# ivanalberico/End-To-End-Self-Supervised-SLAM

Measured on AMD Instinct MI355X. Metric: online refinement steps/sec @640x480, seq_len=60, higher is better.
Workload: dtype f32

## Files before the change

### end-to-end-self-supervised-slam_amd/csrc/conv.hip

```cpp
#include <cassert>
#include <type_traits>

#include "e2e_common.h"

typedef float f4v __attribute__((ext_vector_type(4)));
typedef float f16v __attribute__((ext_vector_type(16)));

#define CBK 16

enum { ACT_NONE = 0, ACT_RELU = 1, ACT_ELU = 2, ACT_DISP = 3 };

struct ConvArgs {
    const float* src0;
    const float* src1;
    const float* w;
    const float* scale;
    const float* shift;
    const float* res;
    float* out;
    int B, Hs, Ws;
    int Cin, C1, up;
    int Hd, Wd;
    int Ncols, ldw;
    int KH, KW, stride, pad, pad_mode;
// ... 1655 lines not shown
#pragma unroll
            for (int mt = 0; mt < MT; ++mt) av[mt] = ap[ks * 4 * CO + mt * 16];
#pragma unroll
            for (int t = 0; t < 9; ++t) {
                const float bv = bp[((t / 3) * PW + (t % 3)) * 16 + ks * 64];
#pragma unroll
                for (int mt = 0; mt < MT; ++mt) acc[mt * 10 + t] = __builtin_amdgcn_mfma_f32_16x16x4f32(av[mt], bv, acc[mt * 10 + t], 0, 0, 0);
            }
#pragma unroll
            for (int mt = 0; mt < MT; ++mt) acc[mt * 10 + 9] = __builtin_amdgcn_mfma_f32_16x16x4f32(av[mt], one, acc[mt * 10 + 9], 0, 0, 0);
        }
    }
    float* red = smem;
    static_assert(2 * NA * 4 * 64 <= PH * PW * 16 + TH * TW * CO, "reduction scratch");
    __syncthreads();
    if (wave >= 2) {
#pragma unroll
        for (int t = 0; t < NA; ++t)
#pragma unroll
            for (int i = 0; i < 4; ++i) red[((wave - 2) * NA * 4 + t * 4 + i) * 64 + lane] = acc[t][i];
    }
    __syncthreads();
    if (wave < 2) {
#pragma unroll
        for (int t = 0; t < NA; ++t)
#pragma unroll
            for (int i = 0; i < 4; ++i) acc[t][i] += red[(wave * NA * 4 + t * 4 + i) * 64 + lane];
    }
    __syncthreads();
    if (wave == 1) {
#pragma unroll
        for (int t = 0; t < NA; ++t)
#pragma unroll
            for (int i = 0; i < 4; ++i) red[(t * 4 + i) * 64 + lane] = acc[t][i];
    }
    __syncthreads();
    if (wave != 0) return;
    const int64_t sid = ((int64_t)b * gridDim.y + blockIdx.y) * a.nxg + blockIdx.x;
    float* slab = a.slabs + sid * CO * a.npad;
    const int kconv = 9 * a.Cin, cg0 = hf * 16;
#pragma unroll
    for (int mt = 0; mt < MT; ++mt)
#pragma unroll
        for (int t = 0; t < 10; ++t)
#pragma unroll
            for (int i = 0; i < 4; ++i) {
                const float v = acc[mt * 10 + t][i] + red[((mt * 10 + t) * 4 + i) * 64 + lane];
                const int co = mt * 16 + 4 * kq + i;
                if (t < 9) slab[co * a.npad + t * a.Cin + cg0 + l16] = v;
                else if (a.has_bias && hf == 0 && l16 == 0) slab[co * a.npad + kconv] = v;
            }
}

struct StemWgradArgs {
    const float* dz;
    const float* src;
    float* slabs;
    int B, Hs, Ws, Hd, Wd, tiles_x, nxg;
    float in_sub, in_mul;
};

__global__ __launch_bounds__(256) void k_wgrad7x7_stem(StemWgradArgs a) {
    constexpr int TH = 4, TW = 32, PH = 2 * TH + 6, PW = 2 * TW + 5, ROW = 208, NPAD = 148;
    __shared__ float patch[PH * ROW];
    __shared__ float dzs[TH * TW * 64];
    const int tid = threadIdx.x, lane = tid & 63, wave = tid >> 6, l16 = lane & 15, kq = lane >> 4;
    const int y0 = blockIdx.y * TH, b = blockIdx.z;
    int offn[10];
#pragma unroll
    for (int nt = 0; nt < 10; ++nt) {
        const int k = 16 * nt + l16;
        offn[nt] = k + (k / 21) * (ROW - 21) + 48 * kq;
    }
    f4v acc[10];
#pragma unroll
    for (int nt = 0; nt < 10; ++nt) acc[nt] = (f4v){0.f, 0.f, 0.f, 0.f};
    const float* sb = a.src + (int64_t)b * a.Hs * a.Ws * 3;
    const float* zb = a.dz + (int64_t)b * a.Hd * a.Wd * 64;
    for (int tx = 0; tx < a.tiles_x; ++tx) {
        const int x0 = (blockIdx.x * a.tiles_x + tx) * TW;
        if (x0 >= a.Wd) break;
        __syncthreads();
        for (int idx = tid; idx < PH * ROW; idx += 256) {
            const int py = idx / ROW, e = idx - py * ROW;
            const int Y = 2 * y0 - 3 + py, X = 2 * x0 - 3 + e / 3;
            const bool ok = e < 3 * PW && Y >= 0 && Y < a.Hs && X >= 0 && X < a.Ws;
            patch[idx] = ok ? (sb[((int64_t)Y * a.Ws + X) * 3 + (e - (e / 3) * 3)] - a.in_sub) * a.in_mul : 0.f;
        }
        for (int idx = tid; idx < TH * TW * 16; idx += 256) {
            const int q = idx & 15, pix = idx >> 4;
            const int r = pix / TW, x = pix - r * TW;
            const bool ok = y0 + r < a.Hd && x0 + x < a.Wd;
            *(f4v*)&dzs[pix * 64 + q * 4] = ok ? *(const f4v*)(zb + ((int64_t)(y0 + r) * a.Wd + x0 + x) * 64 + q * 4) : (f4v){0.f, 0.f, 0.f, 0.f};
        }
        __syncthreads();
#pragma unroll 1
        for (int r = 0; r < TH; ++r) {
            const float* ap = dzs + (r * TW + 8 * kq) * 64 + 16 * wave + l16;
            const float* bp = patch + 2 * r * ROW;
#pragma unroll 2
            for (int ks = 0; ks < TW / 4; ++ks) {
                const float av = ap[ks * 64];
#pragma unroll
                for (int nt = 0; nt < 10; ++nt) acc[nt] = __builtin_amdgcn_mfma_f32_16x16x4f32(av, bp[offn[nt] + ks * 6], acc[nt], 0, 0, 0);
            }
        }
// ... 632 lines not shown
#pragma unroll
            for (int kw = 0; kw < 3; ++kw) {
                const float* wt = &sw[(kh * 3 + kw) * HC + cq * 4];
                const float gg = head_dz_gather(gz, h, ww, kh, kw, H, W, rya, ryb, rxa, rxb);
#pragma unroll
                for (int c = 0; c < 4; ++c) da[c] = fmaf(gg, wt[c], da[c]);
            }
        if (dact) {
#pragma unroll
            for (int e = 0; e < 4; ++e) da[e] *= act_deriv(xv[e], dact);
        }
        *(f4v*)(dx + n * HC + cq * 4) = da;
    }
#pragma unroll
    for (int k = 0; k < 36; ++k) {
        float v = acc[k];
#pragma unroll
        for (int o = 4; o < 64; o <<= 1) v += __shfl_xor(v, o, 64);
        acc[k] = v;
    }
#pragma unroll
    for (int o = 4; o < 64; o <<= 1) sb += __shfl_xor(sb, o, 64);
    if (lane < 4) {
#pragma unroll
        for (int t = 0; t < 9; ++t)
#pragma unroll
            for (int c = 0; c < 4; ++c) red[wave][t * HC + lane * 4 + c] = acc[t * 4 + c];
        if (lane == 0) red[wave][9 * HC] = sb;
    }
    __syncthreads();
    if (threadIdx.x < 9 * HC + 1)
        partials[(int64_t)blockIdx.x * (9 * HC + 1) + threadIdx.x] = ((red[0][threadIdx.x] + red[1][threadIdx.x]) + red[2][threadIdx.x]) + red[3][threadIdx.x];
}

__global__ __launch_bounds__(256) void k_head_wreduce(const float* __restrict__ partials, int nparts, float* __restrict__ dw, float* __restrict__ dbias) {
    __shared__ float red[4];
    const int col = blockIdx.x;
    float s = 0.f;
    for (int i = threadIdx.x; i < nparts; i += 256) s += partials[(int64_t)i * (9 * HC + 1) + col];
    const float t = block_sum(s, red);
    if (threadIdx.x == 0) {
        if (col == 9 * HC) { if (dbias) dbias[0] = t; }
        else { const int tap = col / HC, ci = col - tap * HC; dw[ci * 9 + tap] = t; }
    }
}

static inline int egrid(int64_t n) { int64_t g = (n + 255) / 256; return (int)(g < 1 ? 1 : (g > 4096 ? 4096 : g)); }

struct GemmCfg { int bm, bn, S; };
#define WGRAD_TARGET 1024

#define CONV_TILE_SHAPES(X)                                                                                      \
    X(64, 64, 2, 2, 1, 1, 32) X(128, 64, 2, 2, 2, 1, 32) X(128, 128, 2, 2, 2, 2, 16) X(128, 32, 4, 1, 1, 1, 32) \
    X(32, 128, 1, 4, 1, 1, 32) X(32, 64, 1, 2, 1, 1, 32) X(64, 32, 2, 1, 1, 1, 32) X(32, 32, 1, 1, 1, 1, 32)
static int tile_max_cb(int bm, int bn) {
#define X(BM, BN, WM, WN, TM, TN, MAXCB) if (bm == BM && bn == BN) return MAXCB;
    CONV_TILE_SHAPES(X)
#undef X
    return 0;
}
static void demote_cb16_only(GemmCfg& c) { if (tile_max_cb(c.bm, c.bn) == 16) c.bn = 64; }

static GemmCfg choose_cfg(int64_t rows, int cols, int K, int cb, bool allow_split, GemmCfg force = GemmCfg{0, 0, 0}) {
    if (force.bm) { GemmCfg f = force; if (!allow_split && f.S > 1) f.S = 1; if (cb != 16) demote_cb16_only(f); return f; }
    GemmCfg c = {64, 64, 1};
    if (cols >= 128) { c.bm = 32; c.bn = 128; }
    if (cols <= 32) {
        c.bm = 128; c.bn = 32;
        if (((rows + 127) / 128) * ((cols + 31) / 32) < 600) c.bm = 64;
    }
    if (allow_split && cols > 32) {
        const int64_t tiles = ((rows + c.bm - 1) / c.bm) * ((cols + c.bn - 1) / c.bn);
        const int nchunks = (K + cb - 1) / cb;
        const int depth = nchunks * cb / 32;
        int S = tiles >= 500 ? 1 : depth < 30 ? 1 : depth < 60 ? 3 : depth < 120 ? 4 : 6;
        while (S < 12 && tiles * S < 200 && (nchunks / (S + 1)) * cb >= 288) ++S;
        while (S > 1 && tiles * S > 1300) --S;
        while (S > 1 && (nchunks / S) * cb < 288) --S;
        if (S < 1) S = 1;
        auto model = [&](int s) {
            const double wgs = (double)tiles * s, per_cu = wgs <= 256 ? 1 : wgs <= 512 ? 2 : wgs <= 768 ? 3 : 0;
            const double f = per_cu == 1 ? 1.0 : per_cu == 2 ? 1.76 : per_cu == 3 ? 2.41 : 2.41 * wgs / 768.0;
            return f * ((double)nchunks / s + 6.0) + (s > 1 ? 4.0 : 0.0);
        };
        if (tiles < 500 && S > 1) {
            int best = S;
            for (int s = S - 2; s <= S + 2; ++s) {
                if (s < 2 || s > 12 || s == S || (nchunks / s) * cb < 288 || tiles * s > 1300) continue;
                if (model(s) < 0.93 * model(best)) best = s;
            }
            S = best;
        }
        c.S = S;
    }
    return c;
}

template <bool TR>
static void launch_tile(ConvArgs& a, int cb, GemmCfg c, dim3 g, hipStream_t st) {
#define X(BM, BN, WM, WN, TM, TN, MAXCB)                                                                                                 \
    if (c.bm == BM && c.bn == BN) {                                                                                                      \
        if constexpr (MAXCB == 32)                                                                                                       \
            if (cb == 32) { hipLaunchKernelGGL((k_conv_gemm<WM, WN, TM, TN, 4, TR, 32>), g, dim3(64 * WM * WN), 0, st, a); return; }     \
        hipLaunchKernelGGL((k_conv_gemm<WM, WN, TM, TN, 4, TR, 16>), g, dim3(64 * WM * WN), 0, st, a);                                   \
        return;                                                                                                                          \
    }
    CONV_TILE_SHAPES(X)
#undef X
    assert(!"launch_tile: shape not in CONV_TILE_SHAPES");
}

template <bool TR>
static void launch_streamk(ConvArgs& a, int cb, int G, float* workspace, hipStream_t st) {
    const int64_t Ntot = (int64_t)a.B * a.Hd * a.Wd;
    SkArgs s;
    s.flags = (unsigned*)workspace;
    s.slabs = workspace + SK_FLAG_FLOATS;
    s.tiles_n = (a.Ncols + 63) / 64;
    s.C = a.KH * a.KW * a.Cin / cb;
    s.I = ((Ntot + 63) / 64) * s.tiles_n * (long long)s.C;
    if (G > SK_MAX_G) G = SK_MAX_G;
    if ((long long)G > s.I) G = (int)s.I;
    s.G = G;
    if (cb == 32) hipLaunchKernelGGL((k_conv_gemm_sk<TR, 32>), dim3(G), dim3(256), 0, st, a, s);
    else hipLaunchKernelGGL((k_conv_gemm_sk<TR, 16>), dim3(G), dim3(256), 0, st, a, s);
}

enum GemmKind { GK_SCALAR, GK_STREAMK, GK_TILE };
enum GemmTail { GT_NONE, GT_SPLITK4, GT_SPLITK, GT_CLS };
struct GemmLaunch { GemmKind kind; GemmTail tail; GemmCfg c; int cb; dim3 g; int G; };

#define CLS_TAP_SLICES 4
static int64_t cls_rows(int B, int Hd, int Wd) { return (int64_t)B * ((Hd + 1) / 2) * ((Wd + 1) / 2); }
static int64_t cls_slab_floats(int B, int Hd, int Wd, int cols) { return CLS_TAP_SLICES * 4 * cls_rows(B, Hd, Wd) * cols; }

template <bool TR>
static GemmLaunch plan_gemm(ConvArgs& a, int vec, float* workspace_all, GemmCfg force) {
    GemmLaunch p{GK_TILE, GT_NONE, GemmCfg{0, 0, 0}, 16, dim3(1), 0};
    const int64_t Ntot = (int64_t)a.B * a.Hd * a.Wd;
    const int K = a.KH * a.KW * a.Cin;
    const int cb = (vec == 4 && a.Cin % 32 == 0 && (a.C1 == a.Cin || a.C1 % 32 == 0)) ? 32 : 16;
    float* workspace = workspace_all ? workspace_all + SK_FLAG_FLOATS : nullptr;
    a.ksplit = 1; a.cps = 0; a.slab = workspace;
    a.bytes0 = (int64_t)a.B * (a.Hs / a.up) * (a.Ws / a.up) * a.C1 * 4;
    a.bytes1 = (int64_t)a.B * a.Hs * a.Ws * (a.Cin - a.C1) * 4;
    a.bytesw = (int64_t)K * a.ldw * 4;
// ... 509 lines not shown
        return p;
    if (vec == 4 && stride == 1 && pad == 1 && Ho == Hs && Wo == Ws && (up == 1 || up == 2) && Hs % up == 0 && Ws % up == 0 && (C1 == Cin || (has_src1 && C1 % 32 == 0)) &&
        getenv("E2E_WGRAD_TAPS") != nullptr && getenv("E2E_WGRAD_TAPS")[0] == '1' && (p = plan(WP_TAPS)).open)
        return p;
    return lean && (p = plan(WP_GEMM16)).open ? p : plan(lean ? WP_GEMM_LEAN : WP_GEMM);
}

int64_t e2e_conv2d_wgrad_workspace_floats(int B, int Ho, int Wo, int Cin, int Cout, int KH, int KW, int has_bias) {
    GEOM_WGRAD_QUERY(g);
    return wgrad_workspace_floats(g, has_bias, false, WGRAD_TARGET);
}

struct WgradOut { float* dw; float* dbias; const float* out_scale; int accumulate; e2e_wgrad_reduce_desc* defer; };

static void wgrad_reduce(const WgradArgs& a, const WgradOut& o, int S, int Mpad, int Npad, int zl, hipStream_t st) {
    if (o.defer) {
        *o.defer = e2e_wgrad_reduce_desc{a.slabs, o.dw, o.dbias, o.out_scale, S, Mpad, Npad, a.Cout, a.Cin, a.KH, a.KW, a.has_bias, o.accumulate, zl, 0};
        return;
    }
    const int64_t tq = (int64_t)a.Cout * ((a.Ngemm + 3) / 4);
    if (zl == 8)
        hipLaunchKernelGGL((k_wgrad_reduce<8>), dim3(egrid(tq * 4)), dim3(512), 0, st, a.slabs, S, Mpad, Npad, a.Cout, a.Cin, a.KH, a.KW, a.has_bias, o.dw,
                           o.dbias, o.accumulate, o.out_scale);
    else
        hipLaunchKernelGGL((k_wgrad_reduce<2>), dim3(egrid(tq * 4)), dim3(128), 0, st, a.slabs, S, Mpad, Npad, a.Cout, a.Cin, a.KH, a.KW, a.has_bias, o.dw,
                           o.dbias, o.accumulate, o.out_scale);
}

enum WgradKernel { WK_DONE, WK_GEMM16, WK_GEMM4_32, WK_GEMM4_64, WK_GEMM_32, WK_GEMM_64 };
struct WgradLaunch { WgradKernel k; dim3 g; int Sz; };

static int wgrad_setup(const WgradIn& in, const ConvGeom& g, int wg_target, const WgradOut& o, hipStream_t st, WgradArgs& a, WgradLaunch& L, bool dry = false) {
    const int B = g.B, Cin = g.Cin, Cout = g.Cout, Ho = g.Ho, Wo = g.Wo;
    const bool tuned = wg_target != 0;
    if (!tuned) wg_target = WGRAD_TARGET;
    L = WgradLaunch{WK_DONE, dim3(1), 0};
    E2E_REQUIRE(in.dz && in.src0 && o.dw && in.workspace && B > 0 && Cin > 0 && Cout > 0, E2E_ERR_ARG, "e2e_conv2d_bwd_weight: bad argument");
    const int vec = (Cin % 4 == 0 && g.C1 % 4 == 0) ? 4 : 1;
    E2E_REQUIRE(vec == 4 || (g.C1 == Cin && g.up == 1 && g.pad_mode == 0), E2E_ERR_ARG, "e2e_conv2d_bwd_weight: scalar path takes one full-resolution zero-padded source");
    a = WgradArgs{};
    a.dz = in.dz; a.src0 = in.src0; a.src1 = in.src1; a.slabs = in.workspace;
    a.B = B; a.Hs = g.Hs; a.Ws = g.Ws; a.Cin = Cin; a.C1 = g.C1; a.up = g.up; a.Ho = Ho; a.Wo = Wo; a.Cout = Cout;
    a.KH = g.KH; a.KW = g.KW; a.stride = g.stride; a.pad = g.pad; a.pad_mode = g.pad_mode; a.has_bias = o.dbias ? 1 : 0;
    a.Ngemm = g.KH * g.KW * Cin + a.has_bias;
    const WgradPlan p = wgrad_choose(g, a.has_bias, in.src1 != nullptr, tuned, wg_target);
    const int S = (int)p.S;
    if (dry && (p.path == WP_STEM || p.path == WP_THIN || p.path == WP_TAPS)) return E2E_OK;
    if (p.path == WP_STEM) {
        StemWgradArgs ta{in.dz, in.src0, in.workspace, B, g.Hs, g.Ws, Ho, Wo, 2, p.nxg, g.in_sub, g.in_mul};
        hipLaunchKernelGGL(k_wgrad7x7_stem, dim3(p.nxg, p.ny, B), dim3(256), 0, st, ta);
    } else if (p.path == WP_THIN) {
        ThinWgradArgs ta{in.dz, in.src0, in.src1, in.workspace, B, Ho, Wo, Cin, g.C1, g.up, p.Npad, a.has_bias, p.tiles_x, p.nxg};
        const dim3 tg((unsigned)p.nxg, (unsigned)p.ny, (unsigned)(B * (Cin / 16)));
        if (Cout == 32) hipLaunchKernelGGL((k_wgrad3x3_thin<2>), tg, dim3(256), 0, st, ta);
        else hipLaunchKernelGGL((k_wgrad3x3_thin<1>), tg, dim3(256), 0, st, ta);
    } else if (p.path == WP_TAPS) {
        TapWgradArgs ta{in.dz, in.src0, in.src1, in.workspace, B, Ho, Wo, Cin, g.C1, g.up, Cout, g.pad_mode == 1 ? 1 : 0, a.has_bias,
                        p.Mpad, p.Npad, p.ptx, p.pty, p.nchunks, p.cps};
        const dim3 tg((unsigned)(Cin / 32), (unsigned)(Cout / 32), (unsigned)S);
        if (a.has_bias) hipLaunchKernelGGL(k_wgrad3x3_taps<true>, tg, dim3(TAP_NT), 0, st, ta);
        else hipLaunchKernelGGL(k_wgrad3x3_taps<false>, tg, dim3(TAP_NT), 0, st, ta);
    }
    if (p.path == WP_STEM || p.path == WP_THIN || p.path == WP_TAPS) {
        wgrad_reduce(a, o, S, p.Mpad, p.Npad, (p.path == WP_TAPS && S < 8) ? 2 : 8, st);
        return E2E_OK;
    }
    const bool use16 = p.path == WP_GEMM16, lean = p.path != WP_GEMM;
    a.Mpad = p.Mpad; a.Npad = p.Npad;
    a.in_sub = g.in_sub; a.in_mul = g.in_mul; a.vec = vec;
    const int64_t P = (int64_t)B * Ho * Wo;
    const int cbp = lean ? 32 : CBK;
    a.pix_per_slice = ((P + p.S - 1) / p.S + cbp - 1) / cbp * cbp;
    L.Sz = (int)((P + a.pix_per_slice - 1) / a.pix_per_slice);
    L.g = dim3((unsigned)(a.Npad / p.tn), (unsigned)(a.Mpad / p.tm), (unsigned)L.Sz);
    L.k = use16 ? WK_GEMM16 : lean ? (p.tm == 32 ? WK_GEMM4_32 : WK_GEMM4_64) : (p.tm == 32 ? WK_GEMM_32 : WK_GEMM_64);
    return E2E_OK;
}

static void wgrad_launch_gemm(const WgradArgs& a, const WgradLaunch& L, hipStream_t st) {
    const dim3 g = L.g;
    const bool two = a.src1 != nullptr;
    if (L.k == WK_GEMM16) hipLaunchKernelGGL((k_wgrad_gemm16<10, 32>), g, dim3(256), 0, st, a);
    else if (L.k == WK_GEMM4_32 && two) hipLaunchKernelGGL((k_wgrad_gemm4<1, 4, 32, true>), g, dim3(256), 0, st, a);
    else if (L.k == WK_GEMM4_32) hipLaunchKernelGGL((k_wgrad_gemm4<1, 4, 32, false>), g, dim3(256), 0, st, a);
    else if (L.k == WK_GEMM4_64 && two) hipLaunchKernelGGL((k_wgrad_gemm4<2, 2, 32, true>), g, dim3(256), 0, st, a);
    else if (L.k == WK_GEMM4_64) hipLaunchKernelGGL((k_wgrad_gemm4<2, 2, 32, false>), g, dim3(256), 0, st, a);
    else if (L.k == WK_GEMM_32 && a.vec == 4) hipLaunchKernelGGL((k_wgrad_gemm<1, 4, 4>), g, dim3(256), 0, st, a);
    else if (L.k == WK_GEMM_32) hipLaunchKernelGGL((k_wgrad_gemm<1, 4, 1>), g, dim3(256), 0, st, a);
    else if (L.k == WK_GEMM_64 && a.vec == 4) hipLaunchKernelGGL((k_wgrad_gemm<2, 2, 4>), g, dim3(256), 0, st, a);
    else if (L.k == WK_GEMM_64) hipLaunchKernelGGL((k_wgrad_gemm<2, 2, 1>), g, dim3(256), 0, st, a);
}

static int bwd_weight_impl(const WgradIn& in, const ConvGeom& g, const WgradOut& o, void* stream, int wg_target = 0) {
    const hipStream_t st = (hipStream_t)stream;
    WgradArgs a;
    WgradLaunch L;
    const int rc = wgrad_setup(in, g, wg_target, o, st, a, L);
    if (rc != E2E_OK) return rc;
    if (L.k != WK_DONE) {
        wgrad_launch_gemm(a, L, st);
        wgrad_reduce(a, o, L.Sz, a.Mpad, a.Npad, L.Sz >= 8 ? 8 : 2, st);
    }
    E2E_LAUNCH_CHECK("e2e_conv2d_bwd_weight");
    return E2E_OK;
}

int e2e_conv2d_bwd_weight(const float* dz, const float* src0, const float* src1, int C1, int up, float* dw, float* dbias,
// ... 175 lines not shown
```

### end-to-end-self-supervised-slam_amd/csrc/depth_ops.hip

```cpp
#include "e2e_common.h"

#define DT 256

__device__ __forceinline__ unsigned int f2key(float f) {
    const unsigned int b = __float_as_uint(f);
    return (b & 0x80000000u) ? ~b : (b | 0x80000000u);
}
__device__ __forceinline__ float key2f(unsigned int k) {
    return __uint_as_float((k & 0x80000000u) ? (k & 0x7FFFFFFFu) : ~k);
}

#define MED_BINS 2048
struct MedState {
    unsigned int prefix, rank, key, index, count;
};

__device__ unsigned int select_bin(const unsigned int* __restrict__ hist, int nb, unsigned int r, unsigned int* r_in, unsigned int* sh) {
    unsigned int c[8], s = 0;
#pragma unroll
    for (int j = 0; j < 8; ++j) {
        const int i = threadIdx.x * 8 + j;
        c[j] = (i < nb) ? hist[i] : 0u;
        s += c[j];
    }
    unsigned int x = s;
#pragma unroll
    for (int o = 1; o < 64; o <<= 1) {
        const unsigned int y = __shfl_up(x, o, 64);
        if ((threadIdx.x & 63) >= o) x += y;
    }
    __syncthreads();
    if ((threadIdx.x & 63) == 63) sh[2 + (threadIdx.x >> 6)] = x;
    __syncthreads();
    unsigned int woff = 0;
    for (int w = 0; w < (int)(threadIdx.x >> 6); ++w) woff += sh[2 + w];
    const unsigned int excl = woff + x - s;
    if (r >= excl && r < excl + s) {
        unsigned int acc = excl;
#pragma unroll
        for (int j = 0; j < 8; ++j) {
            if (r < acc + c[j]) { sh[0] = threadIdx.x * 8 + j; sh[1] = r - acc; break; }
            acc += c[j];
        }
    }
    __syncthreads();
    *r_in = sh[1];
    return sh[0];
}

template <int PASS, bool RECIP = false>
__global__ __launch_bounds__(DT) void k_median_hist(const float* __restrict__ x, int64_t n, unsigned int rank0,
                                                    unsigned int* __restrict__ hist , MedState* __restrict__ st,
                                                    float* __restrict__ recip_out = nullptr) {
    __shared__ unsigned int lh[MED_BINS];
    __shared__ unsigned int sh[8];
// ... 26 lines not shown
    for (int i = threadIdx.x; i < MED_BINS; i += DT)
        if (lh[i]) atomicAdd(&gh[i], lh[i]);
}

__global__ __launch_bounds__(DT) void k_median_final(const float* __restrict__ x, int64_t n, const unsigned int* __restrict__ hist,
                                                     MedState* __restrict__ st, float* __restrict__ value_out) {
    __shared__ unsigned int sh[8];
    unsigned int rin;
    const unsigned int b2 = select_bin(hist + 2 * MED_BINS, 1024, st->rank, &rin, sh);
    const unsigned int key = st->prefix | b2;
    if (blockIdx.x == 0 && threadIdx.x == 0) { st->key = key; *value_out = key2f(key); }
    for (int64_t i = (int64_t)blockIdx.x * DT + threadIdx.x; i < n; i += (int64_t)gridDim.x * DT)
        if (f2key(x[i]) == key) { atomicMin(&st->index, (unsigned int)i); atomicAdd(&st->count, 1u); }
}

__global__ __launch_bounds__(DT) void k_median_final_scale(const float* __restrict__ delta, int64_t n, const unsigned int* __restrict__ hist,
                                                           MedState* __restrict__ st, const float* __restrict__ m_gt, float* __restrict__ median_out,
                                                           float* __restrict__ depth, float* __restrict__ ratio_out) {
    __shared__ unsigned int sh[8];
    unsigned int rin;
    const unsigned int b2 = select_bin(hist + 2 * MED_BINS, 1024, st->rank, &rin, sh);
    const unsigned int key = st->prefix | b2;
    const float med = key2f(key);
    const float rho = m_gt[0] / med;
    if (blockIdx.x == 0 && threadIdx.x == 0) {
        st->key = key;
        *median_out = med;
        if (ratio_out) ratio_out[0] = rho;
    }
    for (int64_t i = (int64_t)blockIdx.x * DT + threadIdx.x; i < n; i += (int64_t)gridDim.x * DT) {
        const float d = delta[i];
        depth[i] = d * rho;
        if (f2key(d) == key) { atomicMin(&st->index, (unsigned int)i); atomicAdd(&st->count, 1u); }
    }
}

__global__ void k_median_init(unsigned int* hist, MedState* st) {
    for (int i = threadIdx.x; i < 3 * MED_BINS; i += blockDim.x) hist[i] = 0;
    if (threadIdx.x == 0) { st->prefix = 0; st->rank = 0; st->key = 0; st->index = 0xFFFFFFFFu; st->count = 0; }
}

__global__ __launch_bounds__(DT) void k_dot_partials(const float* __restrict__ a, const float* __restrict__ b, int64_t n,
                                                     float* __restrict__ partials) {
    __shared__ float red[DT / 64];
    float acc = 0.f;
    for (int64_t i = (int64_t)blockIdx.x * DT + threadIdx.x; i < n; i += (int64_t)gridDim.x * DT) acc = fmaf(a[i], b[i], acc);
    const float s = block_sum(acc, red);
    if (threadIdx.x == 0) partials[blockIdx.x] = s;
}

__global__ __launch_bounds__(DT) void k_scale_chain_bwd(const float* __restrict__ g, const float* __restrict__ delta,
                                                        const float* __restrict__ m_gt, const float* __restrict__ m_delta,
                                                        const MedState* __restrict__ st, const float* __restrict__ partials,
                                                        int nparts, float* __restrict__ g_disp, int64_t n, const int* __restrict__ elems, int n_elems) {
    __shared__ float sS;
    if (threadIdx.x == 0) {
        double acc = 0.0;
        for (int i = 0; i < nparts; ++i) acc += (double)partials[i];
        sS = (float)acc;
    }
    __syncthreads();
    const float md = m_delta[0], rho = m_gt[0] / md;
    const float corr = -(rho / md) * sS;
    const float share = corr / (float)(n_elems > 0 ? (unsigned int)n_elems : st->count);
    for (int64_t i = (int64_t)blockIdx.x * DT + threadIdx.x; i < n; i += (int64_t)gridDim.x * DT) {
        const float d = delta[i];
        float gd = rho * g[i];
        if (n_elems > 0) {
            for (int e = 0; e < n_elems; ++e) if ((int)i == elems[e]) gd += share;
        } else if (d == md) gd += share;
        g_disp[i] = -(d * d) * gd;
    }
}

__global__ __launch_bounds__(DT) void k_diff_partials(const float* __restrict__ a, const float* __restrict__ b, int64_t n, int kind,
                                                      float* __restrict__ partials) {
    __shared__ float red[DT / 64];
    float acc = 0.f;
    for (int64_t i = (int64_t)blockIdx.x * DT + threadIdx.x; i < n; i += (int64_t)gridDim.x * DT) {
        const float e = a[i] - b[i];
        acc += (kind == 2) ? e * e : fabsf(e);
    }
    const float s = block_sum(acc, red);
    if (threadIdx.x == 0) partials[blockIdx.x] = s;
}

__global__ void k_sum_partials(const float* __restrict__ partials, int nparts, double scale, float* __restrict__ out) {
    __shared__ double sh[4];
    double acc = 0.0;
    for (int i = threadIdx.x; i < nparts; i += blockDim.x) acc += (double)partials[i];
    acc = wave_sum_d(acc);
    if ((threadIdx.x & 63) == 0) sh[threadIdx.x >> 6] = acc;
    __syncthreads();
    if (threadIdx.x == 0) out[0] = (float)((((sh[0] + sh[1]) + sh[2]) + sh[3]) * scale);
}

__global__ __launch_bounds__(DT) void k_diff_bwd(const float* __restrict__ a, const float* __restrict__ b, const float* __restrict__ g,
                                                 int64_t n, int kind, float* __restrict__ gb) {
    const float s = g[0] / (float)n;
    for (int64_t i = (int64_t)blockIdx.x * DT + threadIdx.x; i < n; i += (int64_t)gridDim.x * DT) {
        const float e = a[i] - b[i];
        gb[i] = (kind == 2) ? s * (-2.f * e) : s * ((e > 0.f) ? -1.f : ((e < 0.f) ? 1.f : 0.f));
    }
}

#define NMET 8
__global__ __launch_bounds__(DT) void k_metrics_partials(const float* __restrict__ gt, const float* __restrict__ pred, int64_t n,
                                                         int mask_zero_gt, float* __restrict__ partials) {
    __shared__ float red[DT / 64];
    float acc[NMET] = {0.f, 0.f, 0.f, 0.f, 0.f, 0.f, 0.f, 0.f};
    for (int64_t i = (int64_t)blockIdx.x * DT + threadIdx.x; i < n; i += (int64_t)gridDim.x * DT) {
// ... 24 lines not shown
        for (int i = 0; i < nparts; ++i) acc += (double)partials[threadIdx.x * nparts + i];
        tot[threadIdx.x] = acc;
    }
    __syncthreads();
    if (threadIdx.x < 7) {
        double v = tot[threadIdx.x] / tot[7];
        if (threadIdx.x == 2 || threadIdx.x == 3) v = sqrt(v);
        out[threadIdx.x] = (float)v;
    }
}

__global__ __launch_bounds__(DT) void k_adam(float* __restrict__ p, const float* __restrict__ g, float* __restrict__ m, float* __restrict__ v,
                                             int64_t n, float one_minus_b1, float b2, float one_minus_b2, float step_size,
                                             float bc2_sqrt, float eps, const float* __restrict__ participants,
                                             const float2* __restrict__ schedule, const int* __restrict__ step_counter, int schedule_len) {
    const int64_t n4 = n >> 2;
    const float cnt = participants ? fmaxf(participants[0], 1.f) : 1.f;
    if (schedule) {
        int t = step_counter[0];
        t = t < 1 ? 1 : (t > schedule_len ? schedule_len : t);
        const float2 sc = schedule[t - 1];
        step_size = sc.x;
        bc2_sqrt = sc.y;
    }
    float4* p4 = (float4*)p; const float4* g4 = (const float4*)g; float4* m4 = (float4*)m; float4* v4 = (float4*)v;
    for (int64_t i = (int64_t)blockIdx.x * DT + threadIdx.x; i < n4; i += (int64_t)gridDim.x * DT) {
        float4 pp = p4[i], gg = g4[i], mm = m4[i], vv = v4[i];
        float* pa = (float*)&pp; float* ga = (float*)&gg; float* ma = (float*)&mm; float* va = (float*)&vv;
#pragma unroll
        for (int k = 0; k < 4; ++k) {
            ga[k] = ga[k] / cnt;
            ma[k] = ma[k] + one_minus_b1 * (ga[k] - ma[k]);
            va[k] = va[k] * b2 + one_minus_b2 * (ga[k] * ga[k]);
            const float den = sqrtf(va[k]) / bc2_sqrt + eps;
            pa[k] = pa[k] - step_size * (ma[k] / den);
        }
        p4[i] = pp; m4[i] = mm; v4[i] = vv;
    }
    for (int64_t i = (n4 << 2) + (int64_t)blockIdx.x * DT + threadIdx.x; i < n; i += (int64_t)gridDim.x * DT) {
        const float gi = g[i] / cnt;
        const float mi = m[i] + one_minus_b1 * (gi - m[i]);
        const float vi = v[i] * b2 + one_minus_b2 * (gi * gi);
        m[i] = mi; v[i] = vi;
        p[i] = p[i] - step_size * (mi / (sqrtf(vi) / bc2_sqrt + eps));
    }
}

__global__ void k_adam_advance(int* __restrict__ step_counter) { step_counter[0] += 1; }

static inline int sgrid(int64_t n, int cap = 1024) {
    int64_t g = (n + DT - 1) / DT;
    return (int)(g < 1 ? 1 : (g > cap ? cap : g));
}
#define RED_PARTS 512

extern "C" {

int64_t e2e_median_workspace_bytes(void) { return (3 * MED_BINS + 8) * 4; }

int e2e_median_lower(const float* x, int64_t n, float* value_out, void* workspace, void* stream) {
    E2E_REQUIRE(n > 0 && n < 0xFFFFFFFFll && x && value_out && workspace, E2E_ERR_ARG, "e2e_median_lower: bad argument");
    hipStream_t st = (hipStream_t)stream;
    unsigned int* hist = (unsigned int*)workspace;
    MedState* ms = (MedState*)(hist + 3 * MED_BINS);
    const unsigned int rank = (unsigned int)((n - 1) / 2);
    const int g = sgrid(n, 96);
    hipLaunchKernelGGL(k_median_init, dim3(1), dim3(256), 0, st, hist, ms);
    hipLaunchKernelGGL(k_median_hist<0>, dim3(g), dim3(DT), 0, st, x, n, rank, hist, ms, (float*)nullptr);
    hipLaunchKernelGGL(k_median_hist<1>, dim3(g), dim3(DT), 0, st, x, n, rank, hist, ms, (float*)nullptr);
    hipLaunchKernelGGL(k_median_hist<2>, dim3(g), dim3(DT), 0, st, x, n, rank, hist, ms, (float*)nullptr);
    hipLaunchKernelGGL(k_median_final, dim3(g), dim3(DT), 0, st, x, n, hist, ms, value_out);
    E2E_LAUNCH_CHECK("e2e_median_lower");
    return E2E_OK;
}

int64_t e2e_depth_scale_workspace_bytes(void) { return e2e_median_workspace_bytes() + RED_PARTS * 4 + 64; }

int e2e_depth_scale_fwd(const float* disp, const float* median_gt, float* delta, float* depth, float* median_delta,
                        float* ratio_out, void* workspace, int64_t n, void* stream) {
    E2E_REQUIRE(n > 0 && disp && median_gt && delta && depth && median_delta && workspace, E2E_ERR_ARG, "e2e_depth_scale_fwd: bad argument");
    hipStream_t st = (hipStream_t)stream;
    E2E_REQUIRE(n < 0xFFFFFFFFll, E2E_ERR_ARG, "e2e_depth_scale_fwd: too many elements");
    unsigned int* hist = (unsigned int*)workspace;
    MedState* ms = (MedState*)(hist + 3 * MED_BINS);
    const unsigned int rank = (unsigned int)((n - 1) / 2);
    const int g = sgrid(n, 96);
    hipLaunchKernelGGL(k_median_init, dim3(1), dim3(256), 0, st, hist, ms);
    hipLaunchKernelGGL((k_median_hist<0, true>), dim3(g), dim3(DT), 0, st, disp, n, rank, hist, ms, delta);
    hipLaunchKernelGGL(k_median_hist<1>, dim3(g), dim3(DT), 0, st, (const float*)delta, n, rank, hist, ms, (float*)nullptr);
    hipLaunchKernelGGL(k_median_hist<2>, dim3(g), dim3(DT), 0, st, (const float*)delta, n, rank, hist, ms, (float*)nullptr);
    hipLaunchKernelGGL(k_median_final_scale, dim3(sgrid(n)), dim3(DT), 0, st, (const float*)delta, n, (const unsigned int*)hist, ms, median_gt, median_delta, depth, ratio_out);
    E2E_LAUNCH_CHECK("e2e_depth_scale_fwd");
    return E2E_OK;
}

__global__ __launch_bounds__(DT) void k_fixed_scale_fwd(const float* __restrict__ disp, float scale, float* __restrict__ delta, float* __restrict__ depth,
                                                        int64_t n) {
    for (int64_t i = (int64_t)blockIdx.x * DT + threadIdx.x; i < n; i += (int64_t)gridDim.x * DT) {
        const float d = 1.f / disp[i];
        if (delta) delta[i] = d;
        depth[i] = d * scale;
    }
}
__global__ __launch_bounds__(DT) void k_fixed_scale_bwd(const float* __restrict__ g_depth, const float* __restrict__ disp, float scale,
                                                        float* __restrict__ g_disp, int64_t n) {
    for (int64_t i = (int64_t)blockIdx.x * DT + threadIdx.x; i < n; i += (int64_t)gridDim.x * DT) {
        const float d = 1.f / disp[i];
        g_disp[i] = -(g_depth[i] * scale) * d * d;
    }
}

int e2e_depth_fixed_scale_fwd(const float* disp, float scale, float* delta, float* depth, int64_t n, void* stream) {
    E2E_REQUIRE(n > 0 && disp && depth, E2E_ERR_ARG, "e2e_depth_fixed_scale_fwd: bad argument");
    hipLaunchKernelGGL(k_fixed_scale_fwd, dim3(sgrid(n)), dim3(DT), 0, (hipStream_t)stream, disp, scale, delta, depth, n);
    E2E_LAUNCH_CHECK("e2e_depth_fixed_scale_fwd");
    return E2E_OK;
}

int e2e_depth_fixed_scale_bwd(const float* g_depth, const float* disp, float scale, float* g_disp, int64_t n, void* stream) {
    E2E_REQUIRE(n > 0 && g_depth && disp && g_disp, E2E_ERR_ARG, "e2e_depth_fixed_scale_bwd: bad argument");
    hipLaunchKernelGGL(k_fixed_scale_bwd, dim3(sgrid(n)), dim3(DT), 0, (hipStream_t)stream, g_depth, disp, scale, g_disp, n);
    E2E_LAUNCH_CHECK("e2e_depth_fixed_scale_bwd");
    return E2E_OK;
}

int e2e_depth_scale_bwd(const float* g_depth, const float* delta, const float* median_gt, const float* median_delta,
                        float* g_disp, void* workspace, int64_t n, void* stream) {
    return e2e_depth_scale_bwd_at(g_depth, delta, median_gt, median_delta, nullptr, 0, g_disp, workspace, n, stream);
}

int e2e_depth_scale_bwd_at(const float* g_depth, const float* delta, const float* median_gt, const float* median_delta, const int* elements,
                           int n_elements, float* g_disp, void* workspace, int64_t n, void* stream) {
    E2E_REQUIRE(n > 0 && g_depth && delta && median_gt && median_delta && g_disp && workspace, E2E_ERR_ARG, "e2e_depth_scale_bwd: bad argument");
    E2E_REQUIRE(n_elements >= 0 && n_elements <= 64 && (n_elements == 0 || elements), E2E_ERR_ARG, "e2e_depth_scale_bwd_at: 0..64 named elements");
    hipStream_t st = (hipStream_t)stream;
    const MedState* ms = (const MedState*)((unsigned int*)workspace + 3 * MED_BINS);
    float* parts = (float*)((char*)workspace + e2e_median_workspace_bytes() + 32);
    const int g = sgrid(n, RED_PARTS);
    hipLaunchKernelGGL(k_dot_partials, dim3(g), dim3(DT), 0, st, g_depth, delta, n, parts);
    hipLaunchKernelGGL(k_scale_chain_bwd, dim3(sgrid(n)), dim3(DT), 0, st, g_depth, delta, median_gt, median_delta, ms, parts, g, g_disp, n, elements, n_elements);
    E2E_LAUNCH_CHECK("e2e_depth_scale_bwd");
    return E2E_OK;
}

int e2e_mean_diff_fwd(const float* a, const float* b, int64_t n, int kind, float* out, float* workspace, void* stream) {
    E2E_REQUIRE(n > 0 && a && b && out && workspace && (kind == 1 || kind == 2), E2E_ERR_ARG, "e2e_mean_diff_fwd: bad argument (kind 1 = l1, 2 = l2)");
    hipStream_t st = (hipStream_t)stream;
    const int g = sgrid(n, RED_PARTS);
    hipLaunchKernelGGL(k_diff_partials, dim3(g), dim3(DT), 0, st, a, b, n, kind, workspace);
    hipLaunchKernelGGL(k_sum_partials, dim3(1), dim3(256), 0, st, workspace, g, 1.0 / (double)n, out);
    E2E_LAUNCH_CHECK("e2e_mean_diff_fwd");
    return E2E_OK;
}

int e2e_mean_diff_bwd(const float* a, const float* b, const float* g_out, int64_t n, int kind, float* g_b, void* stream) {
    E2E_REQUIRE(n > 0 && a && b && g_out && g_b && (kind == 1 || kind == 2), E2E_ERR_ARG, "e2e_mean_diff_bwd: bad argument");
    hipLaunchKernelGGL(k_diff_bwd, dim3(sgrid(n)), dim3(DT), 0, (hipStream_t)stream, a, b, g_out, n, kind, g_b);
    E2E_LAUNCH_CHECK("e2e_mean_diff_bwd");
    return E2E_OK;
}

int e2e_depth_metrics(const float* gt, const float* pred, int64_t n, int mask_zero_gt, float* out7, float* workspace, void* stream) {
    E2E_REQUIRE(n > 0 && gt && pred && out7 && workspace, E2E_ERR_ARG, "e2e_depth_metrics: bad argument");
    hipStream_t st = (hipStream_t)stream;
    const int g = sgrid(n, 256);
    hipLaunchKernelGGL(k_metrics_partials, dim3(g), dim3(DT), 0, st, gt, pred, n, mask_zero_gt, workspace);
    hipLaunchKernelGGL(k_metrics_final, dim3(1), dim3(64), 0, st, workspace, g, out7);
    E2E_LAUNCH_CHECK("e2e_depth_metrics");
    return E2E_OK;
}
int64_t e2e_reduce_workspace_floats(void) { return NMET * 256 > RED_PARTS ? NMET * 256 : RED_PARTS; }

int e2e_adam_step(float* params, const float* grads, float* exp_avg, float* exp_avg_sq, int64_t n, float lr, float beta1,
                  float beta2, float eps, int step, void* stream) {
    E2E_REQUIRE(n > 0 && params && grads && exp_avg && exp_avg_sq && step >= 1, E2E_ERR_ARG, "e2e_adam_step: bad argument");
    E2E_REQUIRE(((uintptr_t)params | (uintptr_t)grads | (uintptr_t)exp_avg | (uintptr_t)exp_avg_sq) % 16 == 0, E2E_ERR_ARG,
                "e2e_adam_step: buffers must be 16-byte aligned");
    const double bc1 = 1.0 - pow((double)beta1, step), bc2 = 1.0 - pow((double)beta2, step);
    const float step_size = (float)((double)lr / bc1), bc2_sqrt = (float)sqrt(bc2);
    hipLaunchKernelGGL(k_adam, dim3(sgrid(n >> 2 > 0 ? n >> 2 : 1, 2048)), dim3(DT), 0, (hipStream_t)stream, params, grads, exp_avg,
                       exp_avg_sq, n, 1.0f - beta1, beta2, 1.0f - beta2, step_size, bc2_sqrt, eps, (const float*)nullptr,
                       (const float2*)nullptr, (const int*)nullptr, 0);
    E2E_LAUNCH_CHECK("e2e_adam_step");
    return E2E_OK;
}

int e2e_adam_step_mean(float* params, const float* grad_sums, const float* participants, float* exp_avg, float* exp_avg_sq, int64_t n,
                       float lr, float beta1, float beta2, float eps, int step, void* stream) {
    E2E_REQUIRE(n > 0 && params && grad_sums && participants && exp_avg && exp_avg_sq && step >= 1, E2E_ERR_ARG, "e2e_adam_step_mean: bad argument");
    E2E_REQUIRE(((uintptr_t)params | (uintptr_t)grad_sums | (uintptr_t)exp_avg | (uintptr_t)exp_avg_sq) % 16 == 0, E2E_ERR_ARG,
                "e2e_adam_step_mean: buffers must be 16-byte aligned");
    const double bc1 = 1.0 - pow((double)beta1, step), bc2 = 1.0 - pow((double)beta2, step);
    const float step_size = (float)((double)lr / bc1), bc2_sqrt = (float)sqrt(bc2);
// ... 23 lines not shown
```

Before: 221.9.

## Add register-pipelined thin wgrad kernel, 96-wide conv tiles, staged scale-chain partials

Adds a new 3x3 thin weight-gradient kernel that keeps dz operands in registers loaded through buffer loads and double-buffers the input patch. It reduces across waves through shared memory instead of re-reading from LDS each step, and it is on by default. It also adds 32x96 and 64x96 conv GEMM tile shapes, chosen by default for 65-96 output columns to cut padding waste. Separately, the scale-chain backward kernel now stages the partial sums into shared memory before the serial thread-0 sum. Higher register pressure and the changed tile choices could hurt occupancy or other layer shapes.

Result: faster. 225.5, median of 6 (+1.6%).

```diff
diff --git a/end-to-end-self-supervised-slam_amd/csrc/conv.hip b/end-to-end-self-supervised-slam_amd/csrc/conv.hip
--- a/end-to-end-self-supervised-slam_amd/csrc/conv.hip
+++ b/end-to-end-self-supervised-slam_amd/csrc/conv.hip
@@ -1731,6 +1731,149 @@
             }
 }
 
+template <int MT, bool BIAS>
+__device__ __forceinline__ void wgrad3x3_thin_regs_body(const ThinWgradArgs& a, float* smem) {
+    constexpr int TH = 4, TW = 64, PH = TH + 2, PW = TW + 2, CO = 16 * MT, NA = 10 * MT, PJ = PH + 1;
+    constexpr unsigned OOB = 0x80000000u;
+    static_assert(2 * 10 * 4 * 64 <= PH * PW * 16, "reduction scratch: ten accumulators of two waves");
+    static_assert(TW * 4 == 256 && (PW - TW) * PH * 4 <= 256, "patch loads: one row of 64 pixels per pass, the rest in one");
+    float* patch = smem;
+    const int tid = threadIdx.x, lane = tid & 63, wave = __builtin_amdgcn_readfirstlane(tid >> 6), l16 = lane & 15, kq = lane >> 4;
+    const int nhalf = a.Cin >> 4, n0 = a.C1 >> 4;
+    const int b = blockIdx.z / nhalf, hf = blockIdx.z % nhalf;
+    const bool first = hf < n0;
+    const int sh = first ? (a.up >> 1) : 0, Cs = first ? a.C1 : a.Cin - a.C1, cs0 = (first ? hf : hf - n0) * 16;
+    const int Hs = a.Hd >> sh, Ws = a.Wd >> sh;
+    const int y0 = blockIdx.y * TH;
+    const float* sb = (first ? a.src0 : a.src1) + (int64_t)b * Hs * Ws * Cs + cs0;
+    const int tx0 = blockIdx.x * a.tiles_x;
+    const int ntl = min(a.tiles_x, (a.Wd + TW - 1) / TW - tx0);
+    const int yr = y0 + wave;
+    const __amdgpu_buffer_rsrc_t rz = __builtin_amdgcn_make_buffer_rsrc(
+        (void*)(a.dz + ((int64_t)b * a.Hd + min(yr, a.Hd - 1)) * a.Wd * CO), 0, yr < a.Hd ? a.Wd * CO * 4 : 0, 0x00020000);
+    const unsigned zl = (unsigned)(kq * CO + l16) * 4u;
+    float areg[TW / 4][MT];
+    f4v preg[PJ];
+    auto load_dz = [&](unsigned zo) {
+#pragma unroll
+        for (int ks = 0; ks < TW / 4; ++ks)
+#pragma unroll
+            for (int mt = 0; mt < MT; ++mt)
+                areg[ks][mt] = __builtin_bit_cast(float, __builtin_amdgcn_raw_buffer_load_b32(rz, zo + (unsigned)(ks * 4 * CO + mt * 16) * 4u, 0, 0));
+    };
+    const int pq = tid & 3, ppx = tid >> 2;
+    const int epy = min(tid >> 3, PH - 1), epx = TW + ((tid >> 2) & 1);
+    auto src_row = [&](int py) { return min(max(reflect1(y0 - 1 + py, a.Hd), 0), a.Hd - 1) >> sh; };
+    auto src_col = [&](int X) { return min(max(reflect1(X, a.Wd), 0), a.Wd - 1) >> sh; };
+    const int erow = src_row(epy) * Ws;
+    auto load_patch = [&](int x0) {
+        const int c = src_col(x0 - 1 + ppx) * Cs + pq * 4;
+#pragma unroll
+        for (int j = 0; j < PH; ++j) preg[j] = *(const f4v*)(sb + (int64_t)src_row(j) * Ws * Cs + c);
+        preg[PH] = *(const f4v*)(sb + (int64_t)(erow + src_col(x0 - 1 + epx)) * Cs + pq * 4);
+    };
+    auto store_patch = [&]() {
+#pragma unroll
+        for (int j = 0; j < PH; ++j) *(f4v*)&patch[(j * PW * 4 + tid) * 4] = preg[j];
+        if (tid < PH * 8) *(f4v*)&patch[((epy * PW + epx) * 4 + pq) * 4] = preg[PH];
+    };
+    f4v acc[NA];
+#pragma unroll
+    for (int t = 0; t < NA; ++t) acc[t] = (f4v){0.f, 0.f, 0.f, 0.f};
+    const float one = (l16 == 0) ? 1.f : 0.f;
+    const float* bp = patch + (wave * PW + kq) * 16 + l16;
+    auto sweep = [&](unsigned zn) {
+        float bv[9];
+#pragma unroll
+        for (int t = 0; t < 9; ++t) bv[t] = bp[((t / 3) * PW + (t % 3)) * 16];
+#pragma unroll
+        for (int ks = 0; ks < TW / 4; ++ks) {
+            float bn[9];
+#pragma unroll
+            for (int t = 0; t < 9; ++t) bn[t] = ks + 1 < TW / 4 ? bp[((t / 3) * PW + (t % 3)) * 16 + (ks + 1) * 64] : 0.f;
+#pragma unroll
+            for (int t = 0; t < 9; ++t)
+#pragma unroll
+                for (int mt = 0; mt < MT; ++mt) acc[mt * 10 + t] = __builtin_amdgcn_mfma_f32_16x16x4f32(areg[ks][mt], bv[t], acc[mt * 10 + t], 0, 0, 0);
+            if constexpr (BIAS) {
+#pragma unroll
+                for (int mt = 0; mt < MT; ++mt) acc[mt * 10 + 9] = __builtin_amdgcn_mfma_f32_16x16x4f32(areg[ks][mt], one, acc[mt * 10 + 9], 0, 0, 0);
+            }
+#pragma unroll
+            for (int mt = 0; mt < MT; ++mt)
+                areg[ks][mt] = __builtin_bit_cast(float, __builtin_amdgcn_raw_buffer_load_b32(rz, zn + (unsigned)(ks * 4 * CO + mt * 16) * 4u, 0, 0));
+#pragma unroll
+            for (int t = 0; t < 9; ++t) bv[t] = bn[t];
+            __builtin_amdgcn_sched_barrier(0);
+        }
+    };
+    if (ntl > 0) {
+        load_dz((unsigned)(tx0 * TW * CO) * 4u + zl);
+        load_patch(tx0 * TW);
+        store_patch();
+    }
+    __syncthreads();
+    for (int tx = 0; tx < ntl; ++tx) {
+        const bool more = tx + 1 < ntl;
+        const int xn = (tx0 + tx + 1) * TW;
+        const unsigned zn = more ? (unsigned)(xn * CO) * 4u + zl : OOB;
+        if (more) load_patch(xn);
+        sweep(zn);
+        __syncthreads();
+        if (more) {
+            store_patch();
+            __syncthreads();
+        }
+    }
+    float* red = smem;
+    const int64_t sid = ((int64_t)b * gridDim.y + blockIdx.y) * a.nxg + blockIdx.x;
+    float* slab = a.slabs + sid * CO * a.npad;
+    const int kconv = 9 * a.Cin, cg0 = hf * 16;
+#pragma unroll
+    for (int mt = 0; mt < MT; ++mt) {
+        if (mt > 0) __syncthreads();
+        if (wave >= 2) {
+#pragma unroll
+            for (int t = 0; t < 10; ++t)
+#pragma unroll
+                for (int i = 0; i < 4; ++i) red[((wave - 2) * 40 + t * 4 + i) * 64 + lane] = acc[mt * 10 + t][i];
+        }
+        __syncthreads();
+        if (wave < 2) {
+#pragma unroll
+            for (int t = 0; t < 10; ++t)
+#pragma unroll
+                for (int i = 0; i < 4; ++i) acc[mt * 10 + t][i] += red[(wave * 40 + t * 4 + i) * 64 + lane];
+        }
+        __syncthreads();
+        if (wave == 1) {
+#pragma unroll
+            for (int t = 0; t < 10; ++t)
+#pragma unroll
+                for (int i = 0; i < 4; ++i) red[(t * 4 + i) * 64 + lane] = acc[mt * 10 + t][i];
+        }
+        __syncthreads();
+        if (wave == 0) {
+#pragma unroll
+            for (int t = 0; t < 10; ++t)
+#pragma unroll
+                for (int i = 0; i < 4; ++i) {
+                    const float v = acc[mt * 10 + t][i] + red[(t * 4 + i) * 64 + lane];
+                    const int co = mt * 16 + 4 * kq + i;
+                    if (t < 9) slab[co * a.npad + t * a.Cin + cg0 + l16] = v;
+                    else if (BIAS && l16 == 0) slab[co * a.npad + kconv] = v;
+                }
+        }
+    }
+}
+
+template <int MT>
+__global__ __launch_bounds__(256) __attribute__((amdgpu_waves_per_eu(MT == 1 ? 4 : 2))) void k_wgrad3x3_thin_regs(ThinWgradArgs a) {
+    __shared__ float smem[6 * 66 * 16];
+    if (a.has_bias && blockIdx.z % (a.Cin >> 4) == 0) wgrad3x3_thin_regs_body<MT, true>(a, smem);
+    else wgrad3x3_thin_regs_body<MT, false>(a, smem);
+}
+
 struct StemWgradArgs {
     const float* dz;
     const float* src;
@@ -2469,7 +2612,8 @@
 
 #define CONV_TILE_SHAPES(X)                                                                                      \
     X(64, 64, 2, 2, 1, 1, 32) X(128, 64, 2, 2, 2, 1, 32) X(128, 128, 2, 2, 2, 2, 16) X(128, 32, 4, 1, 1, 1, 32) \
-    X(32, 128, 1, 4, 1, 1, 32) X(32, 64, 1, 2, 1, 1, 32) X(64, 32, 2, 1, 1, 1, 32) X(32, 32, 1, 1, 1, 1, 32)
+    X(32, 128, 1, 4, 1, 1, 32) X(32, 64, 1, 2, 1, 1, 32) X(64, 32, 2, 1, 1, 1, 32) X(32, 32, 1, 1, 1, 1, 32) \
+    X(32, 96, 1, 3, 1, 1, 32) X(64, 96, 2, 3, 1, 1, 32)
 static int tile_max_cb(int bm, int bn) {
 #define X(BM, BN, WM, WN, TM, TN, MAXCB) if (bm == BM && bn == BN) return MAXCB;
     CONV_TILE_SHAPES(X)
@@ -2509,6 +2653,10 @@
             S = best;
         }
         c.S = S;
+    }
+    if (cols > 64 && cols <= 96) {
+        const char* ev = getenv("E2E_TILE96");
+        if (!(ev && ev[0] == '0')) { c.bm = ev && ev[0] == '6' ? 64 : 32; c.bn = 96; }
     }
     return c;
 }
@@ -3124,7 +3272,11 @@
     } else if (p.path == WP_THIN) {
         ThinWgradArgs ta{in.dz, in.src0, in.src1, in.workspace, B, Ho, Wo, Cin, g.C1, g.up, p.Npad, a.has_bias, p.tiles_x, p.nxg};
         const dim3 tg((unsigned)p.nxg, (unsigned)p.ny, (unsigned)(B * (Cin / 16)));
-        if (Cout == 32) hipLaunchKernelGGL((k_wgrad3x3_thin<2>), tg, dim3(256), 0, st, ta);
+        const char* ev = getenv("E2E_THIN_WGRAD_REGS");
+        const bool regs = !(ev && ev[0] == '0') && (int64_t)Wo * Cout * 4 < (1ll << 31);
+        if (regs && Cout == 32) hipLaunchKernelGGL((k_wgrad3x3_thin_regs<2>), tg, dim3(256), 0, st, ta);
+        else if (regs) hipLaunchKernelGGL((k_wgrad3x3_thin_regs<1>), tg, dim3(256), 0, st, ta);
+        else if (Cout == 32) hipLaunchKernelGGL((k_wgrad3x3_thin<2>), tg, dim3(256), 0, st, ta);
         else hipLaunchKernelGGL((k_wgrad3x3_thin<1>), tg, dim3(256), 0, st, ta);
     } else if (p.path == WP_TAPS) {
         TapWgradArgs ta{in.dz, in.src0, in.src1, in.workspace, B, Ho, Wo, Cin, g.C1, g.up, Cout, g.pad_mode == 1 ? 1 : 0, a.has_bias,
diff --git a/end-to-end-self-supervised-slam_amd/csrc/depth_ops.hip b/end-to-end-self-supervised-slam_amd/csrc/depth_ops.hip
--- a/end-to-end-self-supervised-slam_amd/csrc/depth_ops.hip
+++ b/end-to-end-self-supervised-slam_amd/csrc/depth_ops.hip
@@ -1,6 +1,9 @@
+#include <cstdlib>
+
 #include "e2e_common.h"
 
 #define DT 256
+#define RED_PARTS 512
 
 __device__ __forceinline__ unsigned int f2key(float f) {
     const unsigned int b = __float_as_uint(f);
@@ -133,11 +136,18 @@
 __global__ __launch_bounds__(DT) void k_scale_chain_bwd(const float* __restrict__ g, const float* __restrict__ delta,
                                                         const float* __restrict__ m_gt, const float* __restrict__ m_delta,
                                                         const MedState* __restrict__ st, const float* __restrict__ partials,
-                                                        int nparts, float* __restrict__ g_disp, int64_t n, const int* __restrict__ elems, int n_elems) {
+                                                        int nparts, float* __restrict__ g_disp, int64_t n, const int* __restrict__ elems, int n_elems,
+                                                        int stage) {
     __shared__ float sS;
+    __shared__ float sp[RED_PARTS];
+    if (stage) {
+        for (int i = threadIdx.x; i < nparts; i += DT) sp[i] = partials[i];
+        __syncthreads();
+    }
     if (threadIdx.x == 0) {
         double acc = 0.0;
-        for (int i = 0; i < nparts; ++i) acc += (double)partials[i];
+        if (stage) for (int i = 0; i < nparts; ++i) acc += (double)sp[i];
+        else for (int i = 0; i < nparts; ++i) acc += (double)partials[i];
         sS = (float)acc;
     }
     __syncthreads();
@@ -268,7 +278,6 @@
     int64_t g = (n + DT - 1) / DT;
     return (int)(g < 1 ? 1 : (g > cap ? cap : g));
 }
-#define RED_PARTS 512
 
 extern "C" {
 
@@ -354,7 +363,9 @@
     float* parts = (float*)((char*)workspace + e2e_median_workspace_bytes() + 32);
     const int g = sgrid(n, RED_PARTS);
     hipLaunchKernelGGL(k_dot_partials, dim3(g), dim3(DT), 0, st, g_depth, delta, n, parts);
-    hipLaunchKernelGGL(k_scale_chain_bwd, dim3(sgrid(n)), dim3(DT), 0, st, g_depth, delta, median_gt, median_delta, ms, parts, g, g_disp, n, elements, n_elements);
+    const char* ev = getenv("E2E_SCALE_CHAIN_STAGED");
+    const int stage = !(ev && ev[0] == '0');
+    hipLaunchKernelGGL(k_scale_chain_bwd, dim3(sgrid(n)), dim3(DT), 0, st, g_depth, delta, median_gt, median_delta, ms, parts, g, g_disp, n, elements, n_elements, stage);
     E2E_LAUNCH_CHECK("e2e_depth_scale_bwd");
     return E2E_OK;
 }
```
